# PartnershipOnAI/safelife

Measured on AMD Instinct MI355X. Metric: env steps/sec (whole node), 8192x25x25 boards; bit-exact vs C advance_board, higher is better.
Workload: dtype u16

## Files before the change

### safelife_amd/csrc/sl_rowlane.hip

```cpp
#include "sl_device.h"
#include <atomic>
#include <cstddef>
#include <cstring>
#include <type_traits>

#include "sl_kernels.h"
#include "sl_planes.h"

namespace sl {
namespace rl {

typedef u32 u32x4 __attribute__((ext_vector_type(4)));

constexpr int WAVES = 4;

#ifdef SL_TRACE
#define SL_STAMP(i)                                                                     \
    do {                                                                                \
        if ((threadIdx.x & 63) == 0 && reward_t)                                        \
            ((long long *)reward_t)[(blockIdx.x * WAVES + (threadIdx.x >> 6)) * 16 + (i)] = (long long)__builtin_amdgcn_s_memrealtime(); \
    } while (0)
#else
#define SL_STAMP(i) do {} while (0)
#endif
// ... 975 lines not shown
    if (!act_rule(c, action, ly, lx, y1, x1)) return;
    board[img[0]] = (u16)c[0];
    board[img[1]] = (u16)c[1];
    board[img[2]] = (u16)c[2];
    board[img[3]] = (u16)c[3];
}

template <int H, int W>
__device__ __forceinline__ bool recolor_exits_lds(u16 *board, int ly, int lx, const int32_t *exits,
                                                  int exit0, int E, int score, int initial, int required,
                                                  int exit_points, int *n_exits = nullptr, u32 *agent_cell = nullptr) {
    using Gm = Geom<H, W>;
    bool any_can = false;
    int at = -1;
    u32 mine = 0;
    if (ly >= 0) {
        at = Gm::cell(ly, lx);
        const u32 c = board[at];
        int earned = score - initial + (has_exited(c) ? exit_points : 0);
        if (earned < 0) earned = 0;
        const bool can = (c & AGENT) && earned >= required;
        mine = (c & ~EXIT) | (can ? EXIT : 0u);
        board[at] = (u16)mine;
        any_can = can;
    }
    const u16 paint = (u16)(FROZEN | EXIT | (any_can ? COLOR_R : 0u));
    int nx = 0;
    if (exit0 >= 0) {
        const int i = Gm::flat(exit0);
        board[i] = paint;
        if (i == at) mine = paint;
        nx = 1;
    }
    for (int k = 1; k < E; ++k) {
        const int ex = exits[k];
        if (ex >= 0) {
            const int i = Gm::flat(ex);
            board[i] = paint;
            if (i == at) mine = paint;
            ++nx;
        }
    }
    if (n_exits) *n_exits = nx;
    if (agent_cell) *agent_cell = mine;
    return any_can;
}


typedef __attribute__((address_space(1))) const void *glds_src_t;
typedef __attribute__((address_space(3))) void *glds_dst_t;

struct NoPerm {
    static __device__ __forceinline__ int swz_chunk(int s) { return s; }
};

template <int MAX_BYTES, bool SWZ = false, int NW = WAVES, class Perm = NoPerm>
__device__ __forceinline__ void dma_to_lds(const unsigned char *__restrict__ src, unsigned char *dst, int bytes,
                                           int lane, int wave) {
    static_assert(!SWZ || !std::is_same<Perm, NoPerm>::value, "a swizzled move names its geometry");
    const int nv = bytes >> 4;
    constexpr int NCH = (MAX_BYTES + 1023) / 1024;
#pragma unroll
    for (int j = 0; j < (NCH + NW - 1) / NW; ++j) {
        const int c = wave + NW * j;
        const int s = c * 64 + lane;
        if (s < nv)
            __builtin_amdgcn_global_load_lds((glds_src_t)(src + (SWZ ? Perm::swz_chunk(s) : s) * 16),
                                             (glds_dst_t)(dst + c * 1024), 16, 0, 0);
    }
}

template <int H, int W, int NW = WAVES>
__device__ __forceinline__ void load_span(const u16 *__restrict__ src, unsigned char *region, int nbb, int lane, int wave) {
    using Gm = Geom<H, W>;
    const int bytes = nbb * Gm::HW * 2;
    dma_to_lds<Gm::SPAN, Gm::KM != 0, NW, Gm>((const unsigned char *)src, region + Gm::PAD, bytes, lane, wave);
    const int nv = bytes >> 4, rem = (bytes & 15) >> 1;
    if (wave == 0 && lane < rem) ((u16 *)(region + Gm::PAD))[nv * 8 + lane] = src[nv * 8 + lane];
}

__device__ __forceinline__ void store16(u32x4 *p, u32x4 v) { __builtin_nontemporal_store(v, p); }

template <int H, int W>
__device__ __forceinline__ void store_span(u16 *__restrict__ dst, const unsigned char *region, int nbb, int tid) {
    using Gm = Geom<H, W>;
    const int bytes = nbb * Gm::HW * 2;
    const int nv = bytes >> 4;
    u32x4 *d = (u32x4 *)dst;
    const u32x4 *s = (const u32x4 *)(region + Gm::PAD);
    constexpr int NVI = (Gm::SPAN / 16 + 64 * WAVES - 1) / (64 * WAVES);
#pragma unroll
    for (int i = 0; i < NVI; ++i) {
        const int slot = tid + 64 * WAVES * i;
        if (slot < nv) store16(d + Gm::swz_chunk(slot), s[slot]);
    }
    const int rem = (bytes & 15) >> 1;
    if (tid < rem) dst[nv * 8 + tid] = ((const u16 *)s)[nv * 8 + tid];
}


template <int H, int W>
__global__ __launch_bounds__(64 * WAVES, (Geom<H, W>::WAVES_PER_SIMD)) void k_advance_rowlane(const u16 *__restrict__ in, u16 *__restrict__ out,
                                                                int B, const float *__restrict__ spawn_prob,
                                                                int n_steps, const int32_t *__restrict__ n_each,
                                                                const int32_t *__restrict__ n_valid,
                                                                sl_pcg64 *rng, const Jump *__restrict__ jump) {
    using Gm = Geom<H, W>;
    extern __shared__ __attribute__((aligned(16))) unsigned char smem[];
    const int tid = threadIdx.x, lane = tid & 63, wave = tid >> 6;
    if (n_valid) B = min(B, *n_valid);
    const int e0b = blockIdx.x * Gm::NB;
    if (e0b >= B) return;
    const int nbb = min(Gm::NB, B - e0b);
    const LaneMap<H, W> lm(lane);
    const int g = lm.g, r = lm.r, up = lm.up, dn = lm.dn;
    const int gb = wave * Gm::G + g;
    const bool rowl = lane < Gm::NL && gb < nbb;
    const bool live = rowl && lm.real;
    const unsigned e = e0b + (rowl ? gb : 0);
    unsigned char *board = smem + Gm::OFF_BOARD;
    u64 *rng_lds = (u64 *)(smem + Gm::OFF_RNG) + 4 * Gm::G * wave;

    load_span<H, W>(in + (size_t)e0b * Gm::HW, board, nbb, lane, wave);
    if (lane < 4 * Gm::G && wave * Gm::G + (lane >> 2) < nbb)
        rng_lds[lane] = ((const u64 *)(rng + e0b + wave * Gm::G))[lane];
    const double p = live ? (double)spawn_prob[e] : 0.0;
    const int my_n = n_each ? (rowl ? max(0, n_each[e]) : 0) : n_steps;
    int wave_n = my_n;
    if (n_each) {
#pragma unroll
        for (int off = 32; off >= 1; off >>= 1) wave_n = max(wave_n, __shfl_xor(wave_n, off));
    }
    __syncthreads();
    const Consts cst = make_consts();
    const pl::PConsts pcst = pl::make_pconsts();
    RowWords<H, W> b;
#pragma unroll
    for (int k = 0; k < Gm::WS; ++k) b[k] = 0;
    if (rowl) read_row<H, W>(board, gb, r, b);
    for (int s = 0; s < wave_n; ++s) {
        const bool going = s < my_n;
        const bool changed = ca_step<H, W, true, false>(b, live && going, going, up, dn, cst, pcst, rng_lds, live ? g : 0, p, jump);
        if (Gm::VERT == V_SHIFT && s + 1 < wave_n && changed) {
            if (live) write_row<H, W>(board, gb, r, b);
            wave_sync();
            if (rowl && !lm.real) read_row<H, W>(board, gb, r, b);
            wave_sync();
        }
    }
    if (live) write_row<H, W>(board, gb, r, b);
    __syncthreads();
    store_span<H, W>(out + (size_t)e0b * Gm::HW, board, nbb, tid);
    if (lane < 4 * Gm::G && wave * Gm::G + (lane >> 2) < nbb)
        ((u64 *)(rng + e0b + wave * Gm::G))[lane] = rng_lds[lane];
}

template <int H, int W>
__global__ __launch_bounds__(64) void k_advance_small(const u16 *__restrict__ in, u16 *__restrict__ out, int B,
                                                      const float *__restrict__ spawn_prob, int n_steps,
                                                      const int32_t *__restrict__ n_each,
                                                      const int32_t *__restrict__ n_valid, sl_pcg64 *rng,
                                                      const Jump *__restrict__ jump) {
    using Gm = Geom<H, W>;
    constexpr int WS = Gm::WS;
    __shared__ u64 rng_lds[4 * Gm::G];
    const int lane = threadIdx.x;
    if (n_valid) B = min(B, *n_valid);
    const int e0b = blockIdx.x * Gm::G;
    if (e0b >= B) return;
    const int nbb = min(Gm::G, B - e0b);
    const LaneMap<H, W> lm(lane);
    const int g = lm.g, r = lm.r;
    const bool rowl = lane < Gm::NL && g < nbb;
    const bool live = rowl && lm.real;
    const unsigned e = e0b + (rowl ? g : 0);
    RowWords<H, W> b;
    {
        const u16 *row = in + ((size_t)e * H + r) * W;
#pragma unroll
        for (int k = 0; k < WS; ++k) {
// ... 910 lines not shown
    constexpr bool GPK = LEAN && GSH_REG && ONE;
    u32 gsh_reg[GSH_REG ? (GPK ? (WS + 4) / 5 : WS) : 1];
    u32 *gsh_lane = GSH_REG ? gsh_reg : (u32 *)(smem_hi + Gm::OFF_GSH) + (wave * 64 + lane) * WS;
    auto set_goal_words = [&](const RowWords<H, W> &g) {
        if constexpr (GPK) {
            goal_pack_row<H, W>(g, gsh_reg);
        } else {
#pragma unroll
            for (int k = 0; k < WS; ++k) gsh_lane[k] = goal_shift(g[k]);
        }
    };
    constexpr bool GCACHE = LEAN && GSH_REG && ONE;
    static_assert(GCACHE == NOGOALS, "the kernels that keep the cache are the ones without a goal image");
    static_assert(GCACHE == GPK, "the kernels that keep the cache hold the words in its packed form");
    using Gc = GoalCache<H, W>;
    u32 *const gc_block = GCACHE && hot_gcache ? hot_gcache + (size_t)((unsigned)hot_first / Gm::NB + blockIdx.x) * Gc::BLOCK_DWORDS
                                               : nullptr;
    u32 *const gc_flag = gc_block;
    u32 gc_word = 0;
    constexpr bool GOALS_FIRST = Gm::WAVES_PER_SIMD == 4;
    if (GCACHE && gc_flag && T > 0) {
        gc_word = *(const u32 *)gc_flag;
        if (GOALS_FIRST) {
#pragma unroll
            for (int c = 0; c < Gc::X4; ++c) {
                const u32x4 v = *Gc::x4(gc_block, wave, lane, c);
                gsh_reg[4 * c + 0] = v.x;
                gsh_reg[4 * c + 1] = v.y;
                gsh_reg[4 * c + 2] = v.z;
                gsh_reg[4 * c + 3] = v.w;
            }
#pragma unroll
            for (int j = 0; j < Gc::TAIL; ++j) gsh_reg[4 * Gc::X4 + j] = *Gc::tail(gc_block, wave, lane, j);
        }
    }
    bool goals_free = false;
    auto gc_look = [&]() {
        if constexpr (GCACHE) {
            u32 seen = gc_word;
            asm volatile("" : "+v"(seen));
            goals_free = __builtin_amdgcn_readfirstlane(seen) == 1u;
        }
    };
    const int8_t *lds_lut = (const int8_t *)(smem_hi + OFF_LUT_V);
    constexpr bool BASE_IN_GSH = GSH_REG && Gm::GSH_BYTES >= WAVES * 64 * WS * 4;
    unsigned char *base_rows = smem_hi + (BASE_IN_GSH ? Gm::OFF_GSH : Gm::OFF_BASE) + wave * 64 * WS * 4;
    const bool inaction = WRAP && (env.wrap.flags & SL_WRAP_INACTION) != 0;
    constexpr int OFF_INB = BASE_IN_GSH ? Gm::LDS_WRAP_GSHREG : Gm::LDS_WRAP_GSHLDS;
    unsigned char *inb = smem_hi + OFF_INB;
    u64 *irng_lds = (u64 *)(smem_hi + OFF_INB + Gm::REGION) + 4 * Gm::G * wave;
    sl_wrap_state *wst = (sl_wrap_state *)(smem_hi + Gm::OFF_WST);
    const double *mvt = (const double *)(smem_hi + Gm::OFF_MVT);
    const int8_t *__restrict__ lut = env.score_lut + 4096;
    const Consts cst = make_consts();
    const pl::PConsts pcst = pl::make_pconsts();
    const u32 cell_mask = vreg(LDS_LUT ? (SCORE_CELL_MASK & 0x7FFF7FFFu) : SCORE_CELL_MASK), c100 = vreg(0x01000100u);

    SL_STAMP(0);
    const u16 *k_board = hot_board, *k_goals = hot_goals;
    const sl_pcg64 *k_rng = hot_rng;
    const int8_t *k_lut = hot_lut;
    asm volatile("" ::"s"(k_board), "s"(k_goals), "s"(k_rng));
    const sl_env_scalars *const sc = hot_scalars + e;
    int gstatic = sc->goals_static, level = sc->level_idx;
    double p = (double)sc->spawn_prob;
    u32 lut_base = (u32)sc->table_idx * (u32)SCORE_LUT_BYTES;
    static_assert(sizeof(sl_env_scalars) == 64, "record stride");
    sl_env_scalars *const lrec = (sl_env_scalars *)(smem_hi + Gm::OFF_REC) + lq;
    int ly = -1, lx = 0, exit0 = -1, action = 0;
    bool pool_exits = false;
    int pre_i[4] = {0, 0, 0, 0}, pre_y1 = 0, pre_x1 = 0;
    u32 pre_c[4] = {0u, 0u, 0u, 0u};
    bool pre_write = false;
    constexpr bool ARGS_EARLY = Gm::WAVES_PER_SIMD == 4;
    auto fetch_args = [&]() {
        const int a0 = env.time_limit, a1 = env.exit_points, a2 = env.auto_reset, a3 = env.L, a4 = env.level_stride;
        const int a5 = env.B, a6 = env.stream_salt, a7 = env.out_compact;
        const void *p0 = out_rec, *p1 = env.pool_board, *p2 = env.pool_goals, *p3 = env.pool_exit_locs;
        const void *p4 = env.pool_rng, *p5 = env.pool_scalars, *p6 = env.exit_locs;
        asm volatile("" ::"s"(a0), "s"(a1), "s"(a2), "s"(a3), "s"(a4), "s"(T), "s"(p0), "s"(p1), "s"(p2), "s"(p3),
                     "s"(p4), "s"(p5), "s"(p6), "s"(reward_t), "s"(done_t), "s"(xcd_base), "s"(xcd_flag), "s"(a5), "s"(a6), "s"(a7));
    };
    constexpr bool MOVE_LDS = ONE && !WRAP && Gm::WAVES_PER_SIMD == 4;
    if (lwave) {
        ly = hot_scalars[el].agent_row;
        lx = hot_scalars[el].agent_col;
        action = actions[el];
        exit0 = env.exit_locs[(size_t)el * E];
        if (ARGS_EARLY) fetch_args();
        if (MOVE_LDS && T > 0 && lead && ly >= 0) {
            int gi[4];
            act_cells<H, W>(ly, lx, action, pre_i, gi, pre_y1, pre_x1);
        }
        if (!MOVE_LDS && T > 0 && lead && ly >= 0) {
            int gi[4];
            act_cells<H, W>(ly, lx, action, pre_i, gi, pre_y1, pre_x1);
            const u16 *src = k_board + (size_t)el * HW;
            pre_c[0] = src[gi[0]];
            pre_c[1] = src[gi[1]];
            pre_c[2] = src[gi[2]];
            pre_c[3] = src[gi[3]];
        }
        SL_STAMP(14);
        gc_look();
        SL_STAMP(13);
    } else {
        constexpr int DW = WAVES - 1;
        const int dw = wave - 1;
        dma_to_lds<Gm::NB * 32, false, DW>((const unsigned char *)(k_rng + e0b), smem_hi + Gm::OFF_RNG, nbb * 32, lane, dw);
        dma_to_lds<Gm::NB * 64, false, DW>((const unsigned char *)(hot_scalars + e0b), smem_hi + Gm::OFF_REC, nbb * 64, lane, dw);
        if (LDS_LUT && !GCACHE) dma_to_lds<4096, false, DW>((const unsigned char *)k_lut, smem_hi + OFF_LUT_V, 4096, lane, dw);
        load_span<H, W, DW>(k_board + (size_t)e0b * HW, board, nbb, lane, dw);
        gc_look();
        if (!NOGOALS) load_span<H, W, DW>(k_goals + (size_t)e0b * HW, goals, nbb, lane, dw);
        if (LDS_LUT && GCACHE) dma_to_lds<4096, false, DW>((const unsigned char *)k_lut, smem_hi + OFF_LUT_V, 4096, lane, dw);
        if (WRAP) {
            dma_to_lds<Gm::NB * (int)sizeof(sl_wrap_state), false, DW>((const unsigned char *)(env.wrap.state + e0b),
                                                                       smem_hi + Gm::OFF_WST,
                                                                       nbb * (int)sizeof(sl_wrap_state), lane, dw);
            if (env.wrap.flags & SL_WRAP_MOVEMENT)
                dma_to_lds<Gm::MVT_N * 8, false, DW>((const unsigned char *)env.wrap.move_table, smem_hi + Gm::OFF_MVT,
                                                     min(env.wrap.move_table_len & ~1, Gm::MVT_N) * 8, lane, dw);
            if (inaction) {
                load_span<H, W, DW>(env.wrap.inaction_board + (size_t)e0b * HW, inb, nbb, lane, dw);
                dma_to_lds<Gm::NB * 32, false, DW>((const unsigned char *)(env.wrap.inaction_rng + e0b),
                                                   smem_hi + OFF_INB + Gm::REGION, nbb * 32, lane, dw);
            }
        }
    }
    if (!GOALS_FIRST && GCACHE && goals_free && live) {
#pragma unroll
        for (int c = 0; c < Gc::X4; ++c) {
            const u32x4 v = *Gc::x4(gc_block, wave, lane, c);
            gsh_reg[4 * c + 0] = v.x;
            gsh_reg[4 * c + 1] = v.y;
            gsh_reg[4 * c + 2] = v.z;
            gsh_reg[4 * c + 3] = v.w;
        }
#pragma unroll
        for (int j = 0; j < Gc::TAIL; ++j) gsh_reg[4 * Gc::X4 + j] = *Gc::tail(gc_block, wave, lane, j);
    }
    constexpr bool MOVE_BOX = !MOVE_LDS && ONE && !(SPAWN && GSH_REG && Gm::WAVES_PER_SIMD == 4);
    if (!lwave || !ARGS_EARLY) fetch_args();
    if (lwave) SL_STAMP(15);
    typedef __attribute__((address_space(3))) int *lds_int;
    lds_int dirty_flag = (lds_int)(smem + Gm::OFF_GOALS);
    if (tid == 0) *dirty_flag = 0;
    constexpr bool QUEUE_OK = !LEAN || Gm::WAVES_PER_SIMD < 4;
    const bool has_queue = QUEUE_OK && env.finished.capacity > 0;
    const bool hand_over = env.auto_reset || has_queue;
    typedef u32 u32x4_t __attribute__((ext_vector_type(4)));
    u32x4_t *const move_box = (u32x4_t *)(smem_hi + OFF_MOVE_V);
    if (MOVE_BOX && lwave) {
        u32x4_t mv = {0xFFFFu, 0xFFFFu, 0xFFFFu, 0xFFFFu};
        if (lead && ly >= 0) pre_write = act_rule(pre_c, action, ly, lx, pre_y1, pre_x1);
        if (pre_write)
            mv = u32x4_t{(u32)pre_i[0] | (pre_c[0] << 16), (u32)pre_i[1] | (pre_c[1] << 16), (u32)pre_i[2] | (pre_c[2] << 16),
                         (u32)pre_i[3] | (pre_c[3] << 16)};
        if (lead) move_box[lq] = mv;
    }
    SL_STAMP(1);
    if (lwave) asm volatile("s_waitcnt lgkmcnt(0)\n\ts_barrier" ::: "memory");
#ifdef SL_TRACE
    else {
        asm volatile("s_waitcnt vmcnt(0) lgkmcnt(0)" ::: "memory");
        SL_STAMP(13);
        __syncthreads();
    }
#else
    else __syncthreads();
#endif
    SL_STAMP(2);
    if (xcd_flag && wave == 1 && (__builtin_amdgcn_s_getreg(20 | (3 << 11)) & 15u) != (((u32)xcd_base + blockIdx.x) & 7u) &&
        lane == 0)
        __hip_atomic_store(xcd_flag, 1u, __ATOMIC_RELAXED, __HIP_MEMORY_SCOPE_SYSTEM);

    if (MOVE_LDS && T > 0) {
        if (lwave && lead && ly >= 0) {
            pre_c[0] = lboard16[pre_i[0]];
            pre_c[1] = lboard16[pre_i[1]];
            pre_c[2] = lboard16[pre_i[2]];
            pre_c[3] = lboard16[pre_i[3]];
            pre_write = act_rule(pre_c, action, ly, lx, pre_y1, pre_x1);
            if (pre_write) {
                lboard16[pre_i[0]] = (u16)pre_c[0];
                lboard16[pre_i[1]] = (u16)pre_c[1];
                lboard16[pre_i[2]] = (u16)pre_c[2];
                lboard16[pre_i[3]] = (u16)pre_c[3];
            }
        }
        asm volatile("s_waitcnt lgkmcnt(0)\n\ts_barrier" ::: "memory");
    }
    RowWords<H, W> b;
    Elig elig;
#pragma unroll
    for (int k = 0; k < WS; ++k) asm volatile("" : "=v"(b[k]));
    if (GCACHE && goals_free) gstatic = 1;
    if (live && !goals_free) {
        if constexpr (NOGOALS) read_row_global<H, W>(k_goals + (size_t)e * HW + r * W, b);
        else read_row<H, W>(goals, gb, r, b);
        set_goal_words(b);
    }
    if (T > 0 && __ballot(rowl && gstatic == 0)) {
        u32 goal_bits = 0;
        if (live) {
#pragma unroll
            for (int k = 0; k < WS; ++k) goal_bits |= b[k];
        }
        const int restless = group_total<H, W>(live && (goal_bits & 0x00810081u) ? 1 : 0, rowl ? g : 0);
        if (rowl && gstatic == 0 && restless == 0) gstatic = 1;
    }
    if (rlead) box[gb].gstat = gstatic;
    SL_STAMP(3);

    bool any_reset = false;
    auto hand_over_block = [&]() {
        const int any = box[0].any;
        if (any & 1) any_reset = true;
        if ((!LEAN || Gm::WAVES_PER_SIMD < 4) && (any & 2)) {
            const int slot = rowl ? box[gb].qslot : -1;
            if (live && slot >= 0) {
                u16 *dst = env.finished.boards + (size_t)slot * HW + r * W;
#pragma unroll 1
                for (int x = 0; x < W; ++x) dst[x] = board16[Gm::cell(r, x)];
            }
        }
        if (!(any & 1)) return;
        SL_STAMP(13);
        const bool ready_pool = env.pool_ready != nullptr;
        const bool l_reset = lead && box[lq].reset_level >= 0;
        sl_level_scalars lv_pre = {};
        int exit0_pre = -1;
        if (l_reset) {
            lv_pre = env.pool_scalars[box[lq].reset_level];
            exit0_pre = env.pool_exit_locs[(size_t)box[lq].reset_level * E];
        }
        const int new_level = rowl ? box[gb].reset_level : -1;
        const bool mine = live && new_level >= 0;
        if (rowl && new_level >= 0) gstatic = 0;
        if (mine) {
            int r2 = r;
            asm volatile("" : "+v"(r2));
            level = new_level;
            const u64 rng_pre = ((const u64 *)(env.pool_rng + level))[r2 & 3];
            constexpr bool EXIT_PRE = !(WRAP && !SPAWN && ONE && W == 48);
            int32_t exit_pre = -1;
            if constexpr (EXIT_PRE) exit_pre = env.pool_exit_locs[(size_t)level * E + (r2 < E ? r2 : 0)];
            const int table_pre = env.pool_scalars[level].table_idx;
            const float spawn_pre = env.pool_scalars[level].spawn_prob;
            asm volatile("" ::: "memory");
            const u16 *pb = (ready_pool ? env.pool_ready : env.pool_board) + (size_t)level * HW, *pg = env.pool_goals + (size_t)level * HW;
            u16 *gdst = (u16 *)(goals + Gm::PAD) + gb * HW;
            typedef u32 u32_a2 __attribute__((aligned(2)));
            const u16 *rows[2] = {pb + r2 * W, pg + r2 * W};
            u16 *imgs[2] = {board16, gdst};
#pragma unroll
            for (int a = 0; a < 2; ++a) {
                u32 tw[WS];
#pragma unroll
                for (int j = 0; j < W / 2; ++j) tw[j] = *(const u32_a2 *)(rows[a] + 2 * j);
                if (Gm::ODD) tw[WS - 1] = rows[a][W - 1];
                if (NOGOALS && a == 1) {
                    u16 *grow = env.goals + (size_t)e * HW + r2 * W;
#pragma unroll
                    for (int j = 0; j < W / 2; ++j) *(u32_a2 *)(grow + 2 * j) = tw[j];
                    if (Gm::ODD) grow[W - 1] = (u16)tw[WS - 1];
                    RowWords<H, W> gw;
                    words_from_pairs<H, W>(tw, gw);
                    set_goal_words(gw);
                    continue;
                }
#pragma unroll
                for (int j = 0; j < W / 2; ++j) {
                    imgs[a][Gm::cell(r, 2 * j)] = (u16)tw[j];
                    imgs[a][Gm::cell(r, 2 * j + 1)] = (u16)(tw[j] >> 16);
                }
                if (Gm::ODD) imgs[a][Gm::cell(r, W - 1)] = (u16)tw[WS - 1];
            }
            lut_base = (u32)table_pre * (u32)SCORE_LUT_BYTES;
            p = (double)spawn_pre;
            rng_lds[4 * g + (r2 & 3)] = rng_pre;
            if (EXIT_PRE && r2 < E) env.exit_locs[(size_t)e * E + r2] = exit_pre;
            if (r2 + (EXIT_PRE ? H : 0) < E) {
                asm volatile("" ::: "memory");
                const int level2 = box[gb].reset_level;
                for (int k = r2 + (EXIT_PRE ? H : 0); k < E; k += H)
                    env.exit_locs[(size_t)e * E + k] = env.pool_exit_locs[(size_t)level2 * E + k];
            }
            if (!NOGOALS) *dirty_flag = 1;
            if (r2 == 0) box[gb].dirty = 1;
        }
        wave_sync();
        if (mine) {
            if constexpr (!NOGOALS) {
                read_row<H, W>(goals, gb, r, b);
#pragma unroll
                for (int k = 0; k < WS; ++k) gsh_lane[k] = goal_shift(b[k]);
            }
            if (!ready_pool) read_row<H, W>(board, gb, r, b);
        }
        if (!ready_pool) {
            const int s0 = group_total<H, W>(
                mine ? row_score<H, W, LDS_LUT, GPK>(b, gsh_lane, lut, lut_base, lds_lut, cell_mask, c100) : 0, live ? g : 0);
            if (rlead) box[gb].score0 = s0;
        }
        if (rlead) box[gb].gstat = gstatic;
        SL_STAMP(14);
        wg_sync();
        SL_STAMP(15);
        if (lead && box[lq].reset_level >= 0) {
            const int l_level = box[lq].reset_level;
            const int episodes = lrec->episode_idx + 1;
            if (env.stream_salt) {
                u64 hi = lrng[0], lo = lrng[1];
                sl_episode_stream(hi, lo, env.stream_salt + (int)el, episodes);
                lrng[0] = hi;
                lrng[1] = lo;
            }
            pool_exits = true;
            const int32_t *exits = env.pool_exit_locs + (size_t)l_level * E;
            exit0 = exit0_pre;
            const sl_level_scalars lv = lv_pre;
            ly = lv.agent_row;
            lx = lv.agent_col;
            int fresh, open0, exited;
            if (ready_pool) {
                open0 = lv.ready & 1;
                fresh = lv.ready >> 1;
                exited = 0;
            } else {
                fresh = box[lq].score0;
                open0 = recolor_exits_lds<H, W>(lboard16, ly, lx, exits, exit0, E, fresh, lv.initial_points,
                                                lv.required_reset, env.exit_points) ? 1 : 0;
                exited = ly >= 0 ? (has_exited(lboard16[Gm::cell(ly, lx)]) ? 1 : 0) : 0;
            }
            if (WRAP) wrap_reset(wst[lq], ly, lx);
            sl_env_scalars rec;
            rec.agent_row = ly;
            rec.agent_col = lx;
            rec.num_steps = 0;
            rec.old_value = fresh + env.exit_points * exited;
            rec.required_points = lv.required_step;
            rec.initial_points = lv.initial_points;
            rec.table_idx = lv.table_idx;
            rec.level_idx = l_level;
            rec.episode_idx = episodes;
            rec.episode_length = 0;
            rec.episode_reward = 0.0f;
            rec.spawn_prob = lv.spawn_prob;
            rec.goals_static = 0;
            rec.is_active = 1;
            rec.exit_open_at_reset = open0;
            rec.loaded = 1;
            *lrec = rec;
        }
        wg_sync();
    };

    for (int t = 0;; ++t) {
        if (t > 0) {
            wg_sync();
            if (hand_over) hand_over_block();
        }
        if (t >= T) break;
        if (WRAP && (env.wrap.flags & SL_WRAP_SIDE_EFFECT) && !inaction) {
            const u32 *src = env.wrap.pool_baseline + ((size_t)level * H + r) * WS;
#pragma unroll
            for (int k = 0; k < WS; ++k)
                __builtin_amdgcn_global_load_lds((glds_src_t)(src + k), (glds_dst_t)(base_rows + k * 256), 4, 0, 0);
        }
        if (WRAP && inaction) {
            const bool fresh = rowl && ((const sl_env_scalars *)(smem_hi + Gm::OFF_REC))[gb].num_steps == 0;
            if (__ballot(fresh)) {
                if (fresh && live) {
                    read_row<H, W>(board, gb, r, b);
                    write_row<H, W>(inb, gb, r, b);
                }
            }
            if (!MOVE_BOX && !MOVE_LDS) wg_sync();
        }
        if (MOVE_BOX && rlead) {
            const u32x4_t mv = move_box[gb];
            if ((mv.x & 0xFFFFu) != 0xFFFFu) {
                board16[mv.x & 0xFFFFu] = (u16)(mv.x >> 16);
                board16[mv.y & 0xFFFFu] = (u16)(mv.y >> 16);
                board16[mv.z & 0xFFFFu] = (u16)(mv.z >> 16);
                board16[mv.w & 0xFFFFu] = (u16)(mv.w >> 16);
            }
        }
        if (!MOVE_BOX && !MOVE_LDS) {
            if (lwave) {
                if (t == 0) {
                    if (lead && ly >= 0) pre_write = act_rule(pre_c, action, ly, lx, pre_y1, pre_x1);
                    if (pre_write) {
                        lboard16[pre_i[0]] = (u16)pre_c[0];
                        lboard16[pre_i[1]] = (u16)pre_c[1];
                        lboard16[pre_i[2]] = (u16)pre_c[2];
                        lboard16[pre_i[3]] = (u16)pre_c[3];
                    }
                } else if (lead && ly >= 0) {
                    action = actions[(size_t)t * B + el];
                    act_gather<H, W>(lboard16, ly, lx, action);
                }
            }
            wg_sync();
        }
        SL_STAMP(4);
        const bool dyn = rowl && gstatic != 1;
        const int goal_pass = __ballot(dyn) ? 1 : -1;
        const int base_pass = (WRAP && inaction) ? (goal_pass > 0 ? 2 : 1) : -1;
        const int passes = 1 + (goal_pass > 0 ? 1 : 0) + (base_pass > 0 ? 1 : 0);
#pragma nounroll
        for (int pass = 0; pass < passes; ++pass) {
            const bool base = WRAP && pass == base_pass;
            const bool has = rowl && (pass == 0 || base || dyn);
            const bool mine = has && lm.real;
            unsigned char *img = pass == 0 ? board : (base ? inb : goals);
            u64 *const pass_rng = base ? irng_lds : rng_lds;
            u16 *const grow = NOGOALS ? env.goals + (size_t)e * HW + r * W : nullptr;
            const bool global_row = NOGOALS && pass == goal_pass;
            if (has) {
                if (global_row) read_row_global<H, W>(grow, b);
                else read_row<H, W>(img, gb, r, b);
            }
            bool changed = true;
            if constexpr (use_planes<H, W>()) {
                u32 row_changed = 0;
#ifndef SL_TIMING_SKIP
#define SL_TIMING_SKIP 0
#endif
                if (SL_TIMING_SKIP & 1) changed = false;
                else
                changed = ca_step<H, W, SPAWN, false>(b, mine, mine, up, dn, cst, pcst, pass_rng, live ? g : 0, p, jump,
                                                      &row_changed);
            } else {
                constexpr bool COLFIRST = LEAN && !SPAWN && (WS <= 13 || Gm::WAVES_PER_SIMD < 4);
                ca_rows<H, W, SPAWN, COLFIRST>(b, b, elig, up, dn, cst);
                if (!mine) elig.clear();
                if (SPAWN && __ballot(elig.any())) {
                    RowWords<H, W> old;
#pragma unroll
                    for (int k = 0; k < WS; ++k) old[k] = 0;
                    if (mine) read_row<H, W>(img, gb, r, old);
                    resolve_draws<H, W>(old, b, elig, pass_rng, live ? g : 0, p, jump);
                }
            }
            if (base && mine) {
#pragma unroll
                for (int k = 0; k < WS; ++k)
                    ((u32 *)base_rows)[k * 64 + lane] =
                        b[k] & ~(PLAYER | (PLAYER << 16)) & ((Gm::ODD && k == WS - 1) ? 0xFFFFu : 0xFFFFFFFFu);
            }
            if (pass == goal_pass) {
                u32 diff = 0;
                if (mine) {
                    RowWords<H, W> old;
                    if (changed) {
                        if (global_row) read_row_global<H, W>(grow, old);
                        else read_row<H, W>(img, gb, r, old);
                    } else {
#pragma unroll
                        for (int k = 0; k < WS; ++k) old[k] = b[k];
                    }
#pragma unroll
                    for (int k = 0; k < WS; ++k)
                        diff |= ((b[k] ^ old[k]) | (b[k] & 0x00800080u)) & (Gm::vm1(k) * 0xFFFFu);
                }
                const int moved = group_total<H, W>(mine && diff ? 1 : 0, rowl ? g : 0);
                if (has && gstatic == 0) gstatic = moved ? 2 : 1;
                if (mine) {
                    set_goal_words(b);
                    if (!NOGOALS) *dirty_flag = 1;
                }
            }
            if (mine && changed) {
                if (global_row) write_row_global<H, W>(grow, b);
                else write_row<H, W>(img, gb, r, b);
            }
        }
        if (passes > 1) {
            wave_sync();
            if (live) read_row<H, W>(board, gb, r, b);
        }
        SL_STAMP(5);
        const int score_rows = (SL_TIMING_SKIP & 2) ? (int)(b[0] & 1u) : group_total<H, W>(
            live ? row_score<H, W, LDS_LUT, GPK>(b, gsh_lane, lut, lut_base, lds_lut, cell_mask, c100) : 0, live ? g : 0);
        if (rlead) {
            box[gb].score = score_rows;
            box[gb].gstat = gstatic;
            box[gb].dirty = 1;
        }
        int b_initial = 0, b_required = 0, b_old_value = 0, b_steps = 0, b_ep_len = 0;
        float b_ep_rew = 0.0f;
        bool b_active = false;
        if (lead) {
            b_initial = lrec->initial_points;
            b_required = lrec->required_points;
            b_old_value = lrec->old_value;
            b_steps = lrec->num_steps + 1;
            b_ep_len = lrec->episode_length;
            b_ep_rew = lrec->episode_reward;
            b_active = lrec->is_active != 0;
        }
        wg_sync();
        SL_STAMP(6);
        bool done = false;
        float w_reward = 0.0f, w_ep_rew = 0.0f;
        bool w_times_up = false, w_open = false;
        int w_exits = 0;
        if (lwave) {
            if (lane == 0) box[0].any = 0;
            if (lead && !(SL_TIMING_SKIP & 4)) {
                const int score = box[lq].score;
                const int32_t *exits = pool_exits ? env.pool_exit_locs + (size_t)lrec->level_idx * E
                                                  : env.exit_locs + (size_t)el * E;
                const bool active = b_active;
                u32 cell = 0;
                w_open = recolor_exits_lds<H, W>(lboard16, ly, lx, exits, exit0, E, score, b_initial, b_required,
                                                 env.exit_points, WRAP ? &w_exits : nullptr, &cell);
                const int steps = b_steps;
                const bool times_up = steps >= env.time_limit;
                float reward = 0.0f;
                bool success = false;
                done = true;
                if (ly >= 0) {
                    success = has_exited(cell);
                    const int value = score + (success ? env.exit_points : 0);
                    reward = (float)((value - b_old_value) * (active ? 1 : 0));
                    lrec->old_value = value;
                    done = !(cell & AGENT) || times_up;
                }
                const float ep_rew = b_ep_rew + reward;
                const int ep_len = b_ep_len + (active ? 1 : 0);
                const bool ended = done && active;
                lrec->agent_row = ly;
                lrec->agent_col = lx;
                lrec->num_steps = steps;
                lrec->episode_reward = ep_rew;
                lrec->episode_length = ep_len;
                lrec->is_active = active && !done ? 1 : 0;
                w_reward = reward;
                w_times_up = times_up;
                w_ep_rew = ep_rew;
                sl_step_out o;
                o.reward = reward;
                o.done = done;
                o.success = success;
                o.times_up = times_up;
                o.reserved = 0;
                o.episode_reward = ep_rew;
                o.episode_length = ep_len;
                unsigned e3 = el;
                asm volatile("" : "+v"(e3));
                if (env.out_compact)
                    ((unsigned long long *)out_rec)[e3] =
                        (unsigned long long)__float_as_uint(reward) |
                        ((unsigned long long)((done ? 1u : 0u) | ((success ? 1u : 0u) << 8) | ((times_up ? 1u : 0u) << 16)) << 32);
                else out_rec[e3] = o;
#ifndef SL_TRACE
                if (reward_t) reward_t[(size_t)t * B + el] = reward;
                if (done_t) done_t[(size_t)t * B + el] = done;
#endif
                if (hand_over) {
                    int slot = -1, next_level = -1, any = 0;
                    if (has_queue && ended) {
                        slot = atomicAdd(env.finished.count, 1);
                        if (slot < env.finished.capacity) {
                            const u32 flags = (success ? 1u : 0u) | ((times_up ? 1u : 0u) << 8);
                            u32x4 *qdst = (u32x4 *)(env.finished.records + slot);
                            qdst[0] = u32x4{(u32)((int)el + env.finished.env_base), (u32)lrec->level_idx, (u32)steps,
                                            (u32)lrec->episode_idx};
                            qdst[1] = u32x4{__float_as_uint(lrec->spawn_prob), __float_as_uint(ep_rew), (u32)ep_len, flags};
                            any |= 2;
                        } else {
                            slot = -1;
                        }
                    }
                    if (env.auto_reset && done) {
                        next_level = env.pool_next ? env.pool_next[lrec->level_idx] : (lrec->level_idx + env.level_stride) % env.L;
                        any |= 1;
                    }
                    box[lq].qslot = slot;
                    box[lq].reset_level = next_level;
                    if (any) atomicOr(&box[0].any, any);
                }
            }
        }
        if (WRAP) {
            if (env.wrap.flags & SL_WRAP_SIDE_EFFECT) {
                wg_sync();
                int mine = 0;
                asm volatile("s_waitcnt vmcnt(0)" ::: "memory");
                if (live) {
                    read_row<H, W>(board, gb, r, b);
                    mine = row_side_effect<H, W>(b, (const u32 *)base_rows + lane, gsh_lane,
                                                 (env.wrap.flags & SL_WRAP_IGNORE_REWARD_CELLS) != 0,
                                                 vreg(~(PLAYER | (PLAYER << 16))), cst.m1);
                }
                const int side_rows = group_total<H, W>(mine, rowl ? g : 0);
                if (rlead) box[gb].side = side_rows;
                wg_sync();
            }
            if (lead) {
                int side = (env.wrap.flags & SL_WRAP_SIDE_EFFECT) ? box[lq].side : 0;
                if (w_open != (lrec->exit_open_at_reset != 0)) side -= w_exits;
                const double shaped = wrap_step(env.wrap, wst[lq], mvt, w_reward, done, w_times_up, w_ep_rew, ly, lx, side);
                unsigned e4 = el;
                asm volatile("" : "+v"(e4));
                env.wrap.shaped_reward[e4] = shaped;
                if (shaped_t) shaped_t[(size_t)t * B + e4] = shaped;
            }
        }
    }

    if (T < 0) {
        if (lwave) {
            if (lane == 0) box[0].any = 0;
            if (lead) {
                int next = -1;
                if (!reset_mask || reset_mask[el]) {
                    const bool was = lrec->loaded != 0;
                    next = !was ? lrec->level_idx
                                : env.pool_next ? env.pool_next[lrec->level_idx] : (lrec->level_idx + env.level_stride) % env.L;
                    if (!was) lrec->episode_idx -= 1;
                    atomicOr(&box[0].any, 1);
                }
                box[lq].reset_level = next;
                box[lq].qslot = -1;
            }
        }
        wg_sync();
        hand_over_block();
    } else if (T == 0) {
        wg_sync();
    }
    SL_STAMP(7);
    if (lwave) {
        if (lead) {
            lrec->agent_row = ly;
            lrec->agent_col = lx;
            lrec->goals_static = box[lq].gstat;
            if (T >= 0) lrec->loaded = 1;
        }
        wave_sync();
        int lane3 = lane;
        asm volatile("" : "+v"(lane3));
        for (int i = lane3; i < nbb * 4; i += 64)
            ((u32x4 *)(env.scalars + e0b))[i] = ((const u32x4 *)(smem_hi + Gm::OFF_REC))[i];
    }
    const int dirty = *dirty_flag;
    SL_STAMP(8);
    int tid2 = tid;
    asm volatile("" : "+v"(tid2));
    const int lane2 = tid2 & 63, wave2 = tid2 >> 6;
    store_span<H, W>(env.board + (size_t)e0b * HW, board, nbb, tid2);
    if (dirty && !NOGOALS) store_span<H, W>(env.goals + (size_t)e0b * HW, goals, nbb, tid2);
    if (GCACHE && gc_flag && T != 0) {
        bool all_static = !any_reset;
        if (!goals_free) {
            all_static = true;
#pragma unroll
            for (int q = 0; q < Gm::NB; ++q)
                if (q < nbb && box[q].gstat != 1) all_static = false;
            if (all_static && live && (nbb == Gm::NB || e0b + nbb >= env.B)) {
#pragma unroll
                for (int c = 0; c < Gc::X4; ++c)
                    *Gc::x4(gc_block, wave2, lane2, c) = u32x4{gsh_reg[4 * c], gsh_reg[4 * c + 1], gsh_reg[4 * c + 2], gsh_reg[4 * c + 3]};
#pragma unroll
                for (int j = 0; j < Gc::TAIL; ++j) *Gc::tail(gc_block, wave2, lane2, j) = gsh_reg[4 * Gc::X4 + j];
            }
        }
        const bool gc_full = nbb == Gm::NB || e0b + nbb >= env.B;
        if (tid2 == 0) {
            if (!all_static) *gc_flag = 0u;
            else if (!goals_free && gc_full) *gc_flag = 1u;
        }
    }
    if (lane2 < 4 * Gm::G && wave2 * Gm::G + (lane2 >> 2) < nbb)
        ((u64 *)(env.rng + e0b + wave2 * Gm::G))[lane2] = ((const u64 *)(smem_hi + Gm::OFF_RNG) + 4 * Gm::G * wave2)[lane2];
    if (WRAP)
        for (int i = tid2; i < nbb * (int)(sizeof(sl_wrap_state) / 4); i += 64 * WAVES)
            ((u32 *)(env.wrap.state + e0b))[i] = ((const u32 *)wst)[i];
    if (WRAP && inaction && T > 0) {
        store_span<H, W>(env.wrap.inaction_board + (size_t)e0b * HW, inb, nbb, tid2);
        if (lane2 < 4 * Gm::G && wave2 * Gm::G + (lane2 >> 2) < nbb)
            ((u64 *)(env.wrap.inaction_rng + e0b + wave2 * Gm::G))[lane2] =
                ((const u64 *)(smem_hi + OFF_INB + Gm::REGION) + 4 * Gm::G * wave2)[lane2];
    }

    SL_STAMP(9);
#ifdef SL_TRACE
    asm volatile("s_waitcnt vmcnt(0)" ::: "memory");
    SL_STAMP(10);
    if ((threadIdx.x & 63) == 0 && reward_t) {
        long long *tr = (long long *)reward_t + (blockIdx.x * WAVES + (threadIdx.x >> 6)) * 16;
        tr[11] = __builtin_amdgcn_s_getreg(20 | (31 << 11));
        tr[12] = __builtin_amdgcn_s_getreg(4 | (31 << 11));
    }
#endif
    if (!LEAN && (env.obs || env.policy_obs)) {
        int *par = (int *)(smem_hi + Gm::OFF_GSH);
        if (lead) {
            int *pp = par + lq * OBS_PAR_INTS;
            const int32_t *obs_exits = pool_exits ? env.pool_exit_locs + (size_t)lrec->level_idx * E
                                                  : env.exit_locs + (size_t)el * E;
            const int y0 = ly >= 0 ? ly : 0, x0 = ly >= 0 ? lx : 0;
            const int vh = env.view_h, vw = env.view_w;
            pp[0] = pos_mod(y0 - vh / 2, H);
            pp[1] = pos_mod(x0 - vw / 2, W);
            for (int k = 0; k < OBS_MAX_EXITS; ++k) {
                int tv = -1, xk = -1;
                if (k < E) xk = k == 0 ? exit0 : obs_exits[k];
                if (xk >= 0) {
                    const int iy = xk / W, ix = xk - iy * W;
                    int jy = pos_mod(iy - y0 + H / 2, H) - H / 2 + vh / 2;
                    int jx = pos_mod(ix - x0 + W / 2, W) - W / 2 + vw / 2;
                    jy = min(max(jy, 0), vh - 1);
                    jx = min(max(jx, 0), vw - 1);
                    tv = jy * vw + jx;
                }
                pp[2 + k] = tv;
                pp[2 + OBS_MAX_EXITS + k] = xk;
            }
        }
        wg_sync();
        if (env.obs) {
            if (env.n_channels == 15) write_obs_block<H, W, 15>(env, smem, e0b, nbb, tid);
            else if (env.n_channels == 19) write_obs_block<H, W, 19>(env, smem, e0b, nbb, tid);
            else write_obs_block<H, W, 0>(env, smem, e0b, nbb, tid);
        }
        if (env.policy_obs) write_policy_block<H, W>(env, smem, e0b, nbb, tid);
    }
}

#ifndef SL_ROWLANE_PART

__global__ void k_build_score_lut(const int32_t *__restrict__ points_table, int n_tables, int8_t *__restrict__ lut) {
    const int i = blockIdx.x * blockDim.x + threadIdx.x;
    if (i >= n_tables * SCORE_LUT_BYTES) return;
    const int t = i / SCORE_LUT_BYTES, j = i - t * SCORE_LUT_BYTES;
    int idx;
    bool valid;
    if (j < 4096) {
        idx = (j & 0x0EFF) | ((j & 0x100) << 7);
        idx &= ~0x100;
        valid = (j & ~0x0FFD) == 0;
    } else {
        idx = j - 4096;
        valid = (idx & ~0x8EFD) == 0;
    }
    int v = 0;
    if (valid) {
        const bool alive = idx & 1, pushable = idx & 4, destr = idx & 8, frozen = idx & 16, pullable = idx & 0x8000;
        const int gc = (idx >> 5) & 7, col = (idx >> 9) & 7;
        const bool excluded = frozen && !(pullable || pushable || destr);
        v = excluded ? 0 : points_table[t * 72 + gc * 9 + (alive ? col : 8)];
    }
    lut[i] = (int8_t)v;
}

__global__ void k_build_baseline(sl_env_batch env) {
    const int H = env.H, W = env.W, WS = (W + 1) / 2, E = env.E;
    const int i = blockIdx.x * blockDim.x + threadIdx.x;
    if (i >= env.L * H) return;
    const int l = i / H, r = i - l * H;
    const sl_level_scalars lv = env.pool_scalars[l];
    const u16 *pb = env.pool_board + (size_t)l * H * W;
    const int32_t *px = env.pool_exit_locs + (size_t)l * E;
    const bool open = lv.agent_row >= 0 && (pb[lv.agent_row * W + lv.agent_col] & AGENT) && 0 >= lv.required_reset;
    u32 *dst = env.wrap.pool_baseline + (size_t)i * WS;
// ... 330 lines not shown
```

Measured before the change: 1.271 billion.

## Fold next-step action gather into end-of-step barrier and prefetch actions

```diff
diff --git a/safelife_amd/csrc/sl_rowlane.hip b/safelife_amd/csrc/sl_rowlane.hip
--- a/safelife_amd/csrc/sl_rowlane.hip
+++ b/safelife_amd/csrc/sl_rowlane.hip
@@ -2171,6 +2171,8 @@
                      "s"(p4), "s"(p5), "s"(p6), "s"(reward_t), "s"(done_t), "s"(xcd_base), "s"(xcd_flag), "s"(a5), "s"(a6), "s"(a7));
     };
     constexpr bool MOVE_LDS = ONE && !WRAP && Gm::WAVES_PER_SIMD == 4;
+    constexpr bool ACT_AHEAD = !ONE && !WRAP;
+    constexpr bool TWO_BARRIERS = !ONE && !WRAP;
     if (lwave) {
         ly = hot_scalars[el].agent_row;
         lx = hot_scalars[el].agent_col;
@@ -2447,8 +2449,9 @@
     };
 
     for (int t = 0;; ++t) {
-        if (t > 0) {
+        if (!TWO_BARRIERS && t > 0) {
             wg_sync();
+            if (!ONE && t < T) SL_STAMP(3);
             if (hand_over) hand_over_block();
         }
         if (t >= T) break;
@@ -2477,7 +2480,7 @@
                 board16[mv.w & 0xFFFFu] = (u16)(mv.w >> 16);
             }
         }
-        if (!MOVE_BOX && !MOVE_LDS) {
+        if (!MOVE_BOX && !MOVE_LDS && (!TWO_BARRIERS || t == 0)) {
             if (lwave) {
                 if (t == 0) {
                     if (lead && ly >= 0) pre_write = act_rule(pre_c, action, ly, lx, pre_y1, pre_x1);
@@ -2488,9 +2491,13 @@
                         lboard16[pre_i[3]] = (u16)pre_c[3];
                     }
                 } else if (lead && ly >= 0) {
-                    action = actions[(size_t)t * B + el];
+                    if (!ACT_AHEAD) action = actions[(size_t)t * B + el];
+#ifdef SL_TRACE
+                    asm volatile("s_waitcnt vmcnt(0)" : "+v"(action)::"memory");
+#endif
                     act_gather<H, W>(lboard16, ly, lx, action);
                 }
+                if (!ONE) SL_STAMP(13);
             }
             wg_sync();
         }
@@ -2572,6 +2579,10 @@
             if (live) read_row<H, W>(board, gb, r, b);
         }
         SL_STAMP(5);
+        if (ACT_AHEAD) {
+            const int tn = t + 1 < T ? t + 1 : t;
+            action = actions[(size_t)tn * B + el];
+        }
         const int score_rows = (SL_TIMING_SKIP & 2) ? (int)(b[0] & 1u) : group_total<H, W>(
             live ? row_score<H, W, LDS_LUT, GPK>(b, gsh_lane, lut, lut_base, lds_lut, cell_mask, c100) : 0, live ? g : 0);
         if (rlead) {
@@ -2591,6 +2602,7 @@
             b_ep_rew = lrec->episode_reward;
             b_active = lrec->is_active != 0;
         }
+        if (!ONE) SL_STAMP(1);
         wg_sync();
         SL_STAMP(6);
         bool done = false;
@@ -2675,6 +2687,7 @@
                 }
             }
         }
+        if (!ONE) SL_STAMP(2);
         if (WRAP) {
             if (env.wrap.flags & SL_WRAP_SIDE_EFFECT) {
                 wg_sync();
@@ -2698,6 +2711,23 @@
                 asm volatile("" : "+v"(e4));
                 env.wrap.shaped_reward[e4] = shaped;
                 if (shaped_t) shaped_t[(size_t)t * B + e4] = shaped;
+            }
+        }
+        if (TWO_BARRIERS) {
+            const bool more = t + 1 < T;
+            if (lwave) {
+                wave_sync();
+                if (more && box[0].any == 0 && lead && ly >= 0) act_gather<H, W>(lboard16, ly, lx, action);
+                if (more) SL_STAMP(13);
+            }
+            wg_sync();
+            if (more) SL_STAMP(3);
+            if (__builtin_amdgcn_readfirstlane(box[0].any) != 0) {
+                hand_over_block();
+                if (more) {
+                    if (lead && ly >= 0) act_gather<H, W>(lboard16, ly, lx, action);
+                    wg_sync();
+                }
             }
         }
     }
```

Result: no change. 1.275 billion, median of 4 (+0.3%).

## Prefetch epilogue LDS state into registers before hand-over to overlap stores

Applied to the files above, without the earlier changes.

```diff
diff --git a/safelife_amd/csrc/sl_rowlane.hip b/safelife_amd/csrc/sl_rowlane.hip
--- a/safelife_amd/csrc/sl_rowlane.hip
+++ b/safelife_amd/csrc/sl_rowlane.hip
@@ -1081,20 +1081,66 @@
 __device__ __forceinline__ void store16(u32x4 *p, u32x4 v) { __builtin_nontemporal_store(v, p); }
 
 template <int H, int W>
+struct SpanOut {
+    using Gm = Geom<H, W>;
+    static constexpr int NV_MAX = Gm::SPAN / 16;
+    static constexpr int NVI = (NV_MAX + 64 * WAVES - 1) / (64 * WAVES);
+    static constexpr int GRP = NVI < 4 ? NVI : 4;
+    static constexpr int NGRP = (NVI + GRP - 1) / GRP;
+    u32x4 c[GRP];
+    u32 cell;
+
+    __device__ __forceinline__ void fetch(const unsigned char *region, int nbb, int tid, int grp) {
+        const u32x4 *s = (const u32x4 *)(region + Gm::PAD);
+#pragma unroll
+        for (int j = 0; j < GRP; ++j) {
+            const int i = grp * GRP + j;
+            if (i >= NVI) continue;
+            int slot = tid + 64 * WAVES * i;
+            if (64 * WAVES * (i + 1) > NV_MAX) slot = min(slot, NV_MAX - 1);
+            c[j] = s[slot];
+        }
+        if (grp == 0) cell = ((const u16 *)s)[((nbb * Gm::HW * 2) >> 4) * 8 + (tid & 7)];
+    }
+    __device__ __forceinline__ void land(int grp) {
+#pragma unroll
+        for (int j = GRP - 1; j >= 0; --j)
+            if (grp * GRP + j < NVI) asm volatile("" : "+v"(c[j]));
+        if (grp == 0) asm volatile("" : "+v"(cell));
+    }
+    __device__ __forceinline__ void store(u16 *__restrict__ dst, int nbb, int tid, int grp) const {
+        const int bytes = nbb * Gm::HW * 2;
+        const int nv = bytes >> 4;
+        u32x4 *d = (u32x4 *)dst;
+#pragma unroll
+        for (int j = 0; j < GRP; ++j) {
+            const int i = grp * GRP + j;
+            if (i >= NVI) continue;
+            const int slot = tid + 64 * WAVES * i;
+            if (slot < nv) store16(d + Gm::swz_chunk(slot), c[j]);
+        }
+        if (grp == NGRP - 1) {
+            const int rem = (bytes & 15) >> 1;
+            if (tid < rem) dst[nv * 8 + tid] = (u16)cell;
+        }
+    }
+    template <bool AHEAD>
+    __device__ __forceinline__ void run(u16 *__restrict__ dst, const unsigned char *region, int nbb, int tid) {
+#pragma unroll
+        for (int grp = 0; grp < NGRP; ++grp) {
+            if (!AHEAD || grp > 0) {
+                fetch(region, nbb, tid, grp);
+                land(grp);
+            }
+            store(dst, nbb, tid, grp);
+        }
+    }
+};
+
+template <int H, int W>
 __device__ __forceinline__ void store_span(u16 *__restrict__ dst, const unsigned char *region, int nbb, int tid) {
-    using Gm = Geom<H, W>;
-    const int bytes = nbb * Gm::HW * 2;
-    const int nv = bytes >> 4;
-    u32x4 *d = (u32x4 *)dst;
-    const u32x4 *s = (const u32x4 *)(region + Gm::PAD);
-    constexpr int NVI = (Gm::SPAN / 16 + 64 * WAVES - 1) / (64 * WAVES);
-#pragma unroll
-    for (int i = 0; i < NVI; ++i) {
-        const int slot = tid + 64 * WAVES * i;
-        if (slot < nv) store16(d + Gm::swz_chunk(slot), s[slot]);
-    }
-    const int rem = (bytes & 15) >> 1;
-    if (tid < rem) dst[nv * 8 + tid] = ((const u16 *)s)[nv * 8 + tid];
+    SpanOut<H, W> sp;
+    sp.template run<false>(dst, region, nbb, tid);
 }
 
 
@@ -2303,8 +2349,7 @@
     SL_STAMP(3);
 
     bool any_reset = false;
-    auto hand_over_block = [&]() {
-        const int any = box[0].any;
+    auto hand_over_block = [&](const int any, auto &&behind) {
         if (any & 1) any_reset = true;
         if ((!LEAN || Gm::WAVES_PER_SIMD < 4) && (any & 2)) {
             const int slot = rowl ? box[gb].qslot : -1;
@@ -2444,14 +2489,59 @@
             *lrec = rec;
         }
         wg_sync();
+        behind();
     };
 
-    for (int t = 0;; ++t) {
+    SpanOut<H, W> ep_img;
+    constexpr int REC_IT = (Gm::NB * 4 + 63) / 64;
+    u32x4 ep_rec[REC_IT];
+    u64 ep_rng = 0, ep_irng = 0;
+    int ep_any = 0, ep_dirty = 0, ep_gstat = 1;
+    constexpr int WST_WORDS = (int)(sizeof(sl_wrap_state) / 4), WST_IT = WRAP ? (Gm::NB * WST_WORDS + 64 * WAVES - 1) / (64 * WAVES) : 1;
+    u32 ep_wst[WST_IT] = {};
+    int tid2 = tid, lane2 = lane, wave2 = tid >> 6;
+    static_assert(Gm::NB <= 64, "lane q of a wave looks at board q: the leaders, the records' copy and the goal-word cache's ballot");
+    constexpr bool EP_PLAIN = !ONE && !LEAN && !SPAWN && H <= 12;
+    auto epilogue_fetch = [&]() {
+        tid2 = tid;
+        asm volatile("" : "+v"(tid2));
+        lane2 = tid2 & 63;
+        wave2 = tid2 >> 6;
+        if constexpr (EP_PLAIN) return;
+        ep_any = box[0].any;
+        if constexpr (!NOGOALS) ep_dirty = *dirty_flag;
+        if constexpr (GCACHE) ep_gstat = box[min(lane2, Gm::NB - 1)].gstat;
+        ep_rng = ((const u64 *)(smem_hi + Gm::OFF_RNG) + 4 * Gm::G * wave2)[min(lane2, 4 * Gm::G - 1)];
+        if (WRAP && inaction && T > 0)
+            ep_irng = ((const u64 *)(smem_hi + OFF_INB + Gm::REGION) + 4 * Gm::G * wave2)[min(lane2, 4 * Gm::G - 1)];
+#pragma unroll
+        for (int k = 0; k < REC_IT; ++k)
+            ep_rec[k] = ((const u32x4 *)(smem_hi + Gm::OFF_REC))[min(lane2 + 64 * k, Gm::NB * 4 - 1)];
+        if constexpr (WRAP) {
+#pragma unroll
+            for (int k = 0; k < WST_IT; ++k) ep_wst[k] = ((const u32 *)wst)[min(tid2 + 64 * WAVES * k, Gm::NB * WST_WORDS - 1)];
+        }
+        ep_img.fetch(board, nbb, tid2, 0);
+        ep_img.land(0);
+        if constexpr (WRAP) {
+#pragma unroll
+            for (int k = WST_IT - 1; k >= 0; --k) asm volatile("" : "+v"(ep_wst[k]));
+        }
+#pragma unroll
+        for (int k = REC_IT - 1; k >= 0; --k) asm volatile("" : "+v"(ep_rec[k]));
+        if (WRAP) asm volatile("" : "+v"(ep_irng));
+        asm volatile("" : "+v"(ep_rng));
+        if constexpr (GCACHE) asm volatile("" : "+v"(ep_gstat));
+        asm volatile("" : "+v"(ep_any));
+        ep_any = __builtin_amdgcn_readfirstlane(ep_any);
+    };
+
+    for (int t = 0; EP_PLAIN || t < T; ++t) {
         if (t > 0) {
             wg_sync();
-            if (hand_over) hand_over_block();
-        }
-        if (t >= T) break;
+            if (hand_over) hand_over_block(box[0].any, [] {});
+        }
+        if (EP_PLAIN && t >= T) break;
         if (WRAP && (env.wrap.flags & SL_WRAP_SIDE_EFFECT) && !inaction) {
             const u32 *src = env.wrap.pool_baseline + ((size_t)level * H + r) * WS;
 #pragma unroll
@@ -2624,6 +2714,8 @@
                 const bool ended = done && active;
                 lrec->agent_row = ly;
                 lrec->agent_col = lx;
+                lrec->goals_static = box[lq].gstat;
+                lrec->loaded = 1;
                 lrec->num_steps = steps;
                 lrec->episode_reward = ep_rew;
                 lrec->episode_length = ep_len;
@@ -2718,39 +2810,35 @@
                 box[lq].qslot = -1;
             }
         }
+    } else if (T == 0) {
+        if (lead) lrec->loaded = 1;
+    }
+    if constexpr (EP_PLAIN) {
+        if (T <= 0) wg_sync();
+        if (T < 0) hand_over_block(box[0].any, [] {});
+        epilogue_fetch();
+    } else {
         wg_sync();
-        hand_over_block();
-    } else if (T == 0) {
-        wg_sync();
+        epilogue_fetch();
+        if (T != 0 && (hand_over || T < 0) && (ep_any & 3)) hand_over_block(ep_any, epilogue_fetch);
     }
     SL_STAMP(7);
     if (lwave) {
-        if (lead) {
-            lrec->agent_row = ly;
-            lrec->agent_col = lx;
-            lrec->goals_static = box[lq].gstat;
-            if (T >= 0) lrec->loaded = 1;
-        }
-        wave_sync();
-        int lane3 = lane;
-        asm volatile("" : "+v"(lane3));
-        for (int i = lane3; i < nbb * 4; i += 64)
-            ((u32x4 *)(env.scalars + e0b))[i] = ((const u32x4 *)(smem_hi + Gm::OFF_REC))[i];
-    }
-    const int dirty = *dirty_flag;
+#pragma unroll
+        for (int k = 0; k < REC_IT; ++k)
+            if (lane2 + 64 * k < nbb * 4)
+                ((u32x4 *)(env.scalars + e0b))[lane2 + 64 * k] =
+                    EP_PLAIN ? ((const u32x4 *)(smem_hi + Gm::OFF_REC))[lane2 + 64 * k] : ep_rec[k];
+    }
+    const int dirty = EP_PLAIN ? *dirty_flag : ep_dirty;
     SL_STAMP(8);
-    int tid2 = tid;
-    asm volatile("" : "+v"(tid2));
-    const int lane2 = tid2 & 63, wave2 = tid2 >> 6;
-    store_span<H, W>(env.board + (size_t)e0b * HW, board, nbb, tid2);
+    if constexpr (EP_PLAIN) store_span<H, W>(env.board + (size_t)e0b * HW, board, nbb, tid2);
+    else ep_img.template run<true>(env.board + (size_t)e0b * HW, board, nbb, tid2);
     if (dirty && !NOGOALS) store_span<H, W>(env.goals + (size_t)e0b * HW, goals, nbb, tid2);
     if (GCACHE && gc_flag && T != 0) {
         bool all_static = !any_reset;
         if (!goals_free) {
-            all_static = true;
-#pragma unroll
-            for (int q = 0; q < Gm::NB; ++q)
-                if (q < nbb && box[q].gstat != 1) all_static = false;
+            all_static = __ballot(lane2 < nbb && ep_gstat != 1) == 0;
             if (all_static && live && (nbb == Gm::NB || e0b + nbb >= env.B)) {
 #pragma unroll
                 for (int c = 0; c < Gc::X4; ++c)
@@ -2766,15 +2854,19 @@
         }
     }
     if (lane2 < 4 * Gm::G && wave2 * Gm::G + (lane2 >> 2) < nbb)
-        ((u64 *)(env.rng + e0b + wave2 * Gm::G))[lane2] = ((const u64 *)(smem_hi + Gm::OFF_RNG) + 4 * Gm::G * wave2)[lane2];
-    if (WRAP)
-        for (int i = tid2; i < nbb * (int)(sizeof(sl_wrap_state) / 4); i += 64 * WAVES)
-            ((u32 *)(env.wrap.state + e0b))[i] = ((const u32 *)wst)[i];
+        ((u64 *)(env.rng + e0b + wave2 * Gm::G))[lane2] =
+            EP_PLAIN ? ((const u64 *)(smem_hi + Gm::OFF_RNG) + 4 * Gm::G * wave2)[lane2] : ep_rng;
+    if (WRAP) {
+#pragma unroll
+        for (int k = 0; k < WST_IT; ++k)
+            if (tid2 + 64 * WAVES * k < nbb * WST_WORDS)
+                ((u32 *)(env.wrap.state + e0b))[tid2 + 64 * WAVES * k] = EP_PLAIN ? ((const u32 *)wst)[tid2 + 64 * WAVES * k] : ep_wst[k];
+    }
     if (WRAP && inaction && T > 0) {
         store_span<H, W>(env.wrap.inaction_board + (size_t)e0b * HW, inb, nbb, tid2);
         if (lane2 < 4 * Gm::G && wave2 * Gm::G + (lane2 >> 2) < nbb)
             ((u64 *)(env.wrap.inaction_rng + e0b + wave2 * Gm::G))[lane2] =
-                ((const u64 *)(smem_hi + OFF_INB + Gm::REGION) + 4 * Gm::G * wave2)[lane2];
+                EP_PLAIN ? ((const u64 *)(smem_hi + OFF_INB + Gm::REGION) + 4 * Gm::G * wave2)[lane2] : ep_irng;
     }
 
     SL_STAMP(9);
```

New measurement: 1.274 billion before, 1.293 billion after, median of 6. 1.01x the previous value.
